# duanyiqun/DiffusionDepth

Hardware: NVIDIA H100
Metric: depth maps/sec @ KITTI 352x1216, Swin-L, 20 DDIM steps (higher is better)
Workload: dtype f32 (fp32-grade products on wgmma: 3-pass fp16 split, fp32 accumulate)

## Files before the change

### diffusiondepth_b200/csrc/convgen.cuh

```cuda
#pragma once
#include "conv_common.cuh"

namespace dd {

struct GenConvArgs {
  int B, H, W;
  int tiles_x, tiles_y, m_tiles, n_tiles;
  int kc0, kc1;
  int c0_ch;
  int taps;
  int ld_out, ch_off;
  int cout;
  const float* shift;
  float acc_scale;
  int relu;
  int m_valid;
  int stride;
  int add_first;
  int shuffle;
  float* y32;
  const float* add32;
  __half* out_hi;
  __half* out_lo;
  float split_scale;
  int* status;
};

constexpr int GEN_BK = 64;

template <int NT>
struct GenCfg {
  static constexpr int BK = GEN_BK;
  static constexpr int ROW_BYTES = BK * 2;
  static constexpr int A_BYTES = TILE_M * ROW_BYTES;
  static constexpr int B_BYTES = NT * ROW_BYTES;
  static constexpr int STAGE_BYTES = 2 * (A_BYTES + B_BYTES);
  static constexpr int NWG = NT > 128 ? 2 : 1;
  static constexpr int NW = NT / NWG;
  static constexpr int THREADS = 128 * (1 + NWG);
  static constexpr int LD = 20;
  static constexpr int STAGING_BYTES = NWG * 128 * LD * 4;
  static constexpr int STAGES_RAW = (227 * 1024 - 1024 - 512 - STAGING_BYTES) / STAGE_BYTES;
  static constexpr int STAGES = STAGES_RAW > 6 ? 6 : STAGES_RAW;
  static_assert(STAGES >= 2, "stage too large");
  static constexpr int SMEM_BYTES = STAGES * STAGE_BYTES + 1024 + 512 + STAGING_BYTES;
  static_assert(SMEM_BYTES <= 232448, "exceeds the 227 KB dynamic shared memory limit");
  static_assert(NW % 16 == 0 && NT <= 256, "bad N tile");
};

template <int NT>
__global__ void __launch_bounds__((GenCfg<NT>::THREADS), 1)
convgen_wgmma_kernel(const __grid_constant__ CUtensorMap tmA0_hi, const __grid_constant__ CUtensorMap tmA0_lo,
                     const __grid_constant__ CUtensorMap tmA1_hi, const __grid_constant__ CUtensorMap tmA1_lo,
                     const __grid_constant__ CUtensorMap tmB_hi, const __grid_constant__ CUtensorMap tmB_lo,
                     const GenConvArgs p) {
  using C = GenCfg<NT>;
  constexpr int NW = C::NW;
  extern __shared__ uint8_t smem_raw[];
  uint8_t* smem = reinterpret_cast<uint8_t*>((reinterpret_cast<uintptr_t>(smem_raw) + 1023) & ~uintptr_t(1023));
  uint64_t* full_bar = reinterpret_cast<uint64_t*>(smem + C::STAGES * C::STAGE_BYTES);
  uint64_t* empty_bar = full_bar + C::STAGES;
  float* stage_f = reinterpret_cast<float*>(smem + C::STAGES * C::STAGE_BYTES + 512);

  const int warp = threadIdx.x >> 5;
  const int lane = threadIdx.x & 31;
  const int kc_total = p.kc0 + p.kc1;
  const int k_iters = p.taps * kc_total;
  const int num_work = p.m_tiles * p.n_tiles;

  if (threadIdx.x == 0) {
    tma_prefetch_desc(&tmA0_hi);
    tma_prefetch_desc(&tmA0_lo);
    tma_prefetch_desc(&tmB_hi);
    tma_prefetch_desc(&tmB_lo);
    for (int s = 0; s < C::STAGES; ++s) {
      mbar_init(&full_bar[s], 2);
      mbar_init(&empty_bar[s], C::NWG);
    }
    fence_barrier_init();
  }
  __syncthreads();
  auto stage_ptr = [&](int s) { return smem + s * C::STAGE_BYTES; };

  if (warp < 4) {
    if constexpr (C::NWG > 1) setmaxnreg_dec<40>();
    if (warp == 0 || warp == 1) {
      const bool act = (warp == 0);
      const bool leader = elect_one();
      int stage = 0;
      uint32_t phase = 0;
      for (int work = blockIdx.x; work < num_work; work += gridDim.x) {
        const int nt = work % p.n_tiles;
        const int mt = work / p.n_tiles;
        const int tx = mt % p.tiles_x, ty = (mt / p.tiles_x) % p.tiles_y, img = mt / (p.tiles_x * p.tiles_y);
        const int x0 = tx * TILE_W, y0 = ty * TILE_H;
        for (int tap = 0; tap < p.taps; ++tap) {
          const int dy = p.taps == 9 ? tap / 3 - 1 : 0, dx = p.taps == 9 ? tap % 3 - 1 : 0;
          for (int kc = 0; kc < kc_total; ++kc) {
            mbar_wait(&empty_bar[stage], phase ^ 1);
            uint8_t* s = stage_ptr(stage);
            const int ax = x0 * p.stride + dx, ay = y0 * p.stride + dy;
            const int kw = kc < p.kc0 ? kc * C::BK : p.c0_ch + (kc - p.kc0) * C::BK;
            if (leader) {
              if (!act) {
                mbar_arrive_expect_tx(&full_bar[stage], 2 * C::B_BYTES);
                tma_load_3d(s + 2 * C::A_BYTES, &tmB_hi, &full_bar[stage], kw, nt * NT, tap);
                tma_load_3d(s + 2 * C::A_BYTES + C::B_BYTES, &tmB_lo, &full_bar[stage], kw, nt * NT, tap);
              } else if (kc < p.kc0) {
                mbar_arrive_expect_tx(&full_bar[stage], 2 * C::A_BYTES);
                tma_load_4d(s, &tmA0_hi, &full_bar[stage], kc * C::BK, ax, ay, img);
                tma_load_4d(s + C::A_BYTES, &tmA0_lo, &full_bar[stage], kc * C::BK, ax, ay, img);
              } else {
                mbar_arrive_expect_tx(&full_bar[stage], 2 * C::A_BYTES);
                tma_load_4d(s, &tmA1_hi, &full_bar[stage], (kc - p.kc0) * C::BK, ax, ay, img);
                tma_load_4d(s + C::A_BYTES, &tmA1_lo, &full_bar[stage], (kc - p.kc0) * C::BK, ax, ay, img);
              }
            }
            __syncwarp();
            if (++stage == C::STAGES) {
              stage = 0;
              phase ^= 1;
            }
          }
        }
      }
    }
  } else {
    if constexpr (C::NWG > 1) setmaxnreg_inc<232>();
    const int wg = (warp >> 2) - 1;
    const int t = threadIdx.x & 127;
    const int q = t >> 5;
    const int m = t;
    const int r = m >> 4, c = m & 15;
    float* S = stage_f + wg * 128 * C::LD;
    float* T = S + q * 32 * C::LD;
    const uint32_t b_off = static_cast<uint32_t>(wg * NW) * C::ROW_BYTES;
    int stage = 0;
    uint32_t phase = 0;
    bool overflow = false;
    const int cq = p.cout >> 2;
    float acc[2][NW / 2];
    for (int work = blockIdx.x; work < num_work; work += gridDim.x) {
      int prev = -1;
      for (int it = 0; it < k_iters; ++it) {
        mbar_wait(&full_bar[stage], phase);
        const uint32_t sa_hi = smem_u32(stage_ptr(stage));
        const uint32_t sa_lo = sa_hi + C::A_BYTES;
        const uint32_t sb_hi = sa_hi + 2 * C::A_BYTES + b_off;
        const uint32_t sb_lo = sb_hi + C::B_BYTES;
        wgmma_fence();
#pragma unroll
        for (int h = 0; h < 2; ++h) {
          const uint32_t ho = static_cast<uint32_t>(h * 64 * C::ROW_BYTES);
#pragma unroll
          for (int k = 0; k < C::BK / 16; ++k) {
            const uint64_t a_hi = wgmma_desc(sa_hi + ho + k * 32, C::ROW_BYTES);
            const uint64_t a_lo = wgmma_desc(sa_lo + ho + k * 32, C::ROW_BYTES);
            const uint64_t b_hi = wgmma_desc(sb_hi + k * 32, C::ROW_BYTES);
            const uint64_t b_lo = wgmma_desc(sb_lo + k * 32, C::ROW_BYTES);
            wgmma_f16<NW>(acc[h], a_lo, b_hi, (it | k) != 0 ? 1u : 0u);
            wgmma_f16<NW>(acc[h], a_hi, b_lo, 1u);
            wgmma_f16<NW>(acc[h], a_hi, b_hi, 1u);
          }
        }
        wgmma_commit();
        wgmma_wait<1>();
        mbar_arrive_if(&empty_bar[prev < 0 ? 0 : prev], t == 0 && prev >= 0);
        prev = stage;
        if (++stage == C::STAGES) {
          stage = 0;
          phase ^= 1;
        }
      }
      wgmma_wait<0>();
      wgmma_fence_regs(acc[0]);
      wgmma_fence_regs(acc[1]);
      mbar_arrive_if(&empty_bar[prev < 0 ? 0 : prev], t == 0 && prev >= 0);

      const int nt = work % p.n_tiles;
      const int mt = work / p.n_tiles;
      const int tx = mt % p.tiles_x, ty = (mt / p.tiles_x) % p.tiles_y, img = mt / (p.tiles_x * p.tiles_y);
      const int x = tx * TILE_W + c, y = ty * TILE_H + r;
      const bool valid = (x < p.W) && (y < p.H) && (p.m_valid <= 0 || (y * p.W + x) < p.m_valid);
      const uint32_t vmask = __ballot_sync(0xffffffffu, valid);
      const uint32_t row_base = static_cast<uint32_t>(((static_cast<size_t>(img) * p.H + y) * p.W + x) * p.cout);
      const uint32_t row_out = static_cast<uint32_t>(((static_cast<size_t>(img) * p.H + y) * p.W + x) * p.ld_out + p.ch_off);
      const bool xpose_path = (p.out_hi == nullptr);
#pragma unroll
      for (int ci = 0; ci < NW / 16; ++ci) {
        const int n0 = nt * NT + wg * NW + ci * 16;
        if (n0 >= p.cout) break;
        const int nvalid = p.cout - n0;
        named_bar_sync(2 + wg, 128);
        stage_acc_cols<NW, 16, C::LD>(acc[0], S, 0, ci * 2);
        stage_acc_cols<NW, 16, C::LD>(acc[1], S, 64, ci * 2);
        named_bar_sync(2 + wg, 128);
        uint32_t o_lane;
        if (p.shuffle) {
          const int sub = n0 / cq, cc = n0 - sub * cq;
          o_lane = static_cast<uint32_t>(
              ((static_cast<size_t>(img) * (2 * p.H) + (2 * y + (sub >> 1))) * (2 * p.W) + (2 * x + (sub & 1))) * cq + cc);
        } else {
          o_lane = row_base + static_cast<uint32_t>(n0);
        }
        const uint32_t o_out = p.shuffle ? o_lane : row_out + static_cast<uint32_t>(n0);
        if (xpose_path) {
          const int sl = lane & 3;
          const bool col_ok = 4 * sl < nvalid;
          const float4 sh = __ldg(reinterpret_cast<const float4*>(p.shift + n0) + sl);
          uint32_t o[4], oo[4];
          float4 ad[4];
#pragma unroll
          for (int k = 0; k < 4; ++k) {
            const int row = (lane >> 2) + 8 * k;
            o[k] = __shfl_sync(0xffffffffu, o_lane, row) + 4 * sl;
            oo[k] = __shfl_sync(0xffffffffu, o_out, row) + 4 * sl;
            ad[k] = (p.add32 && col_ok && ((vmask >> row) & 1u)) ? __ldg(reinterpret_cast<const float4*>(p.add32 + o[k]))
                                                                  : make_float4(0.f, 0.f, 0.f, 0.f);
          }
#pragma unroll
          for (int k = 0; k < 4; ++k) {
            const int row = (lane >> 2) + 8 * k;
            if (!((vmask >> row) & 1u) || !col_ok) continue;
            const float4 a4 = *reinterpret_cast<const float4*>(T + row * C::LD + 4 * sl);
            float tt[4] = {fmaf(a4.x, p.acc_scale, sh.x), fmaf(a4.y, p.acc_scale, sh.y), fmaf(a4.z, p.acc_scale, sh.z),
                           fmaf(a4.w, p.acc_scale, sh.w)};
            const float av[4] = {ad[k].x, ad[k].y, ad[k].z, ad[k].w};
#pragma unroll
            for (int j = 0; j < 4; ++j) {
              if (p.add_first) tt[j] += av[j];
              if (p.relu == 1) tt[j] = fmaxf(tt[j], 0.f);
              else if (p.relu == 2) tt[j] = 0.5f * tt[j] * (1.f + erff(tt[j] * 0.70710678118654752f));
              else if (p.relu == 3) tt[j] = tt[j] * fminf(fmaxf(tt[j] + 3.f, 0.f), 6.f) * (1.f / 6.f);
              if (!p.add_first) tt[j] += av[j];
            }
            if (p.y32) *reinterpret_cast<float4*>(p.y32 + oo[k]) = make_float4(tt[0], tt[1], tt[2], tt[3]);
          }
        } else if (valid) {
          float v[16];
#pragma unroll
          for (int j4 = 0; j4 < 4; ++j4) {
            const float4 sh = __ldg(reinterpret_cast<const float4*>(p.shift + n0) + j4);
            const float4 a4 = *reinterpret_cast<const float4*>(S + m * C::LD + 4 * j4);
// ... 9 lines not shown
                const float4 a = __ldg(reinterpret_cast<const float4*>(p.add32 + o_lane) + j4);
                v[4 * j4] += a.x; v[4 * j4 + 1] += a.y; v[4 * j4 + 2] += a.z; v[4 * j4 + 3] += a.w;
              }
            }
          }
          if (p.relu == 1) {
#pragma unroll
            for (int j = 0; j < 16; ++j) v[j] = fmaxf(v[j], 0.f);
          } else if (p.relu == 2) {
#pragma unroll
            for (int j = 0; j < 16; ++j) v[j] = 0.5f * v[j] * (1.f + erff(v[j] * 0.70710678118654752f));
          } else if (p.relu == 3) {
#pragma unroll
            for (int j = 0; j < 16; ++j) v[j] = v[j] * fminf(fmaxf(v[j] + 3.f, 0.f), 6.f) * (1.f / 6.f);
          }
          if (p.add32 && !p.add_first) {
#pragma unroll
            for (int j4 = 0; j4 < 4; ++j4) {
              if (4 * j4 < nvalid) {
                const float4 a = __ldg(reinterpret_cast<const float4*>(p.add32 + o_lane) + j4);
                v[4 * j4] += a.x; v[4 * j4 + 1] += a.y; v[4 * j4 + 2] += a.z; v[4 * j4 + 3] += a.w;
              }
            }
          }
          if (p.y32) {
            float4* d4 = reinterpret_cast<float4*>(p.y32 + o_out);
#pragma unroll
            for (int j = 0; j < 4; ++j)
              if (4 * j < nvalid) d4[j] = make_float4(v[4 * j], v[4 * j + 1], v[4 * j + 2], v[4 * j + 3]);
          }
          __align__(16) __half2 hi[8];
          __align__(16) __half2 lo[8];
          float amax = 0.f;
#pragma unroll
          for (int j = 0; j < 8; ++j) {
            const float s0 = v[2 * j] * p.split_scale, s1 = v[2 * j + 1] * p.split_scale;
            amax = fmaxf(amax, fmaxf(fabsf(s0), fabsf(s1)));
            hi[j] = __floats2half2_rn(s0, s1);
            const float2 back = __half22float2(hi[j]);
            lo[j] = __floats2half2_rn(s0 - back.x, s1 - back.y);
          }
          overflow |= !(amax <= 60000.f);
          uint4* dh = reinterpret_cast<uint4*>(p.out_hi + o_out);
          uint4* dl = reinterpret_cast<uint4*>(p.out_lo + o_out);
#pragma unroll
          for (int j = 0; j < 2; ++j) {
            if (8 * j < nvalid) {
              dh[j] = reinterpret_cast<const uint4*>(hi)[j];
              dl[j] = reinterpret_cast<const uint4*>(lo)[j];
            }
          }
        }
      }
    }
    if (overflow) atomicOr(p.status, 1);
  }
}

__global__ void nchw_to_nhwc_split_kernel(const float* __restrict__ in, __half* __restrict__ hi, __half* __restrict__ lo,
                                          int C, int P, float scale, int* status) {
  __shared__ float t[32][33];
  const int b = blockIdx.z;
  const int p0 = blockIdx.x * 32, c0 = blockIdx.y * 32;
  const float* src = in + static_cast<size_t>(b) * C * P;
  for (int i = threadIdx.y; i < 32; i += blockDim.y) {
    const int c = c0 + i, pp = p0 + threadIdx.x;
    t[i][threadIdx.x] = (c < C && pp < P) ? src[static_cast<size_t>(c) * P + pp] : 0.f;
  }
  __syncthreads();
  bool ov = false;
  for (int i = threadIdx.y; i < 32; i += blockDim.y) {
    const int pp = p0 + i, c = c0 + threadIdx.x;
    if (pp < P && c < C) {
      const float s = t[threadIdx.x][i] * scale;
      ov |= fabsf(s) > 60000.f;
      const __half h = __float2half_rn(s);
      const size_t o = (static_cast<size_t>(b) * P + pp) * C + c;
      hi[o] = h;
      lo[o] = __float2half_rn(s - __half2float(h));
    }
  }
  if (ov) atomicOr(status, 1);
}

__global__ void rgb_to_planes_kernel(const float* __restrict__ rgb, __half* __restrict__ hi, __half* __restrict__ lo,
                                     int B, int HW, float scale, int* status) {
  const size_t n = static_cast<size_t>(B) * HW;
  bool ov = false;
  for (size_t i = blockIdx.x * static_cast<size_t>(blockDim.x) + threadIdx.x; i < n * GEN_BK;
       i += static_cast<size_t>(gridDim.x) * blockDim.x) {
    const int c = static_cast<int>(i % GEN_BK);
    const size_t px = i / GEN_BK;
    float v = 0.f;
    if (c < 3) {
      const size_t b = px / HW, p = px % HW;
      v = rgb[(b * 3 + c) * HW + p] * scale;
    }
    ov |= fabsf(v) > 60000.f;
    const __half h = __float2half_rn(v);
    hi[i] = h;
    lo[i] = __float2half_rn(v - __half2float(h));
  }
  if (ov) atomicOr(status, 1);
}

__global__ void adaptive_avg_pool_nhwc_kernel(const float* __restrict__ in, float* __restrict__ out, int B, int IH, int IW,
// ... 65 lines not shown
```

### diffusiondepth_b200/csrc/engine.cu

```cuda
#include <cuda.h>
#include <cuda_runtime.h>
#include <math.h>
#include <stdio.h>
#include <stdlib.h>
#include <string.h>

#include <algorithm>
#include <map>
#include <string>
#include <vector>

#include "../../include/dd_engine.h"
#include "kernels.cuh"
#include "convgen.cuh"
#include "conv_halo.cuh"
#include "pred_fold.cuh"
#include "swin.cuh"
#include "mpvit.cuh"
#include "backward.cuh"

namespace {

thread_local std::string g_err;

// ... 1267 lines not shown
    if ((rc = bn_fold(bn, cout_conv, scale, shift, st))) return rc;
  } else if (bias) {
    CUDA_TRY(cudaMemcpyAsync(shift.data(), bias, cout_conv * 4, cudaMemcpyDeviceToHost, st));
    CUDA_TRY(cudaStreamSynchronize(st));
  }
  const int cp = cin_pad > 0 ? cin_pad : cin;
  L.cin = cp;
  L.taps = transposed ? 1 : taps;
  L.cout = transposed ? 4 * cout_conv : cout_conv;
  L.shuffle = transposed ? 1 : 0;
  L.relu = 1;
  L.nt = 64;
  if (nt > 0) {
    if (nt != 64 && nt != 128 && nt != 192 && nt != 256) return fail(DD_ERR_INVALID, "N tile must be 64, 128, 192 or 256");
    L.nt = nt;
  } else if (L.cout > 64) {
    int best = 1 << 30;
    for (int width : {256, 192, 128}) {
      const int padded = (L.cout + width - 1) / width * width;
      if (padded < best) { best = padded; L.nt = width; }
    }
  }
  if (L.cout % 8 != 0 || cp % 8 != 0) return fail(DD_ERR_UNSUPPORTED, "channels must be multiples of 8: " + name);
  const int cout_pad = (L.cout + L.nt - 1) / L.nt * L.nt;
  const size_t n = static_cast<size_t>(L.cout) * cp * L.taps;
  float* d_scale = nullptr;
  if ((rc = dev_alloc(owned, reinterpret_cast<void**>(&L.w_hi), n * 2))) return rc;
  if ((rc = dev_alloc(owned, reinterpret_cast<void**>(&L.w_lo), n * 2))) return rc;
  if ((rc = dev_alloc(owned, reinterpret_cast<void**>(&L.shift), cout_pad * 4))) return rc;
  if (bn) {
    if ((rc = dev_alloc(owned, reinterpret_cast<void**>(&d_scale), cout_conv * 4))) return rc;
    CUDA_TRY(cudaMemcpyAsync(d_scale, scale.data(), cout_conv * 4, cudaMemcpyHostToDevice, st));
  }
  if (cp != cin) {
    CUDA_TRY(cudaMemsetAsync(L.w_hi, 0, n * 2, st));
    CUDA_TRY(cudaMemsetAsync(L.w_lo, 0, n * 2, st));
  }
  std::vector<float> shift_full(cout_pad, 0.f);
  for (int i = 0; i < L.cout; ++i) shift_full[i] = shift[i % cout_conv];
  CUDA_TRY(cudaMemcpyAsync(L.shift, shift_full.data(), cout_pad * 4, cudaMemcpyHostToDevice, st));
  if (gen_parts(L.taps, gen_chunks(cp) + 1) > 1) {
    if ((rc = dev_alloc(owned, reinterpret_cast<void**>(&L.zero_shift), cout_pad * 4))) return rc;
    CUDA_TRY(cudaMemsetAsync(L.zero_shift, 0, cout_pad * 4, st));
  }
  const int nraw = static_cast<int>(static_cast<size_t>(cout_conv) * cin * (transposed ? 4 : taps));
  if ((rc = split_scale(scratch, st, &L.wscale, [&] {
         dd::absmax_scaled_kernel<<<absmax_grid(nraw), 256, 0, st>>>(w, d_scale, nraw, cin * L.taps, cout_conv,
                                                                     L.shuffle, scratch);
       })))
    return rc;
  dd::pack_gen_weight_kernel<<<256, 256, 0, st>>>(w, d_scale, L.w_hi, L.w_lo, L.cout, cin, L.taps, L.shuffle, L.wscale, cp);
  if ((rc = check_launch("pack_gen_weight"))) return rc;
  CUDA_TRY(cudaStreamSynchronize(st));
  if ((rc = make_weight_map(&L.mb_hi, L.w_hi, L.cout, cp, L.taps, dd::GEN_BK, L.nt))) return rc;
  if ((rc = make_weight_map(&L.mb_lo, L.w_lo, L.cout, cp, L.taps, dd::GEN_BK, L.nt))) return rc;
  L.alt = (L.nt == 256 && L.cout % 256 == 0 && L.cout % 192 == 0 && !L.shuffle);
  if (L.alt) {
    if ((rc = make_weight_map(&L.mb_hi_alt, L.w_hi, L.cout, cp, L.taps, dd::GEN_BK, 192))) return rc;
    if ((rc = make_weight_map(&L.mb_lo_alt, L.w_lo, L.cout, cp, L.taps, dd::GEN_BK, 192))) return rc;
  }
  return DD_OK;
}

int pack_gen(dd_engine* e, GenLayer& L, const std::string& wkey, const std::string& bnkey, int cin, int cout_conv,
             int taps, bool transposed, cudaStream_t st, float* scratch, int cin_pad = 0,
             const std::string& biaskey = std::string()) {
  const Raw* w = find(e, wkey);
  if (!w) return fail(DD_ERR_INVALID, "missing weights: " + wkey);
  const int k = taps == 9 ? 3 : (transposed ? 2 : 1);
  std::vector<int64_t> want = transposed ? std::vector<int64_t>{cin, cout_conv, 2, 2}
                                         : std::vector<int64_t>{cout_conv, cin, k, k};
  if (w->shape != want) return fail(DD_ERR_INVALID, "weight shape mismatch: " + wkey);
  const float* bn[4] = {nullptr, nullptr, nullptr, nullptr};
  const float* bias = nullptr;
  int rc;
  if (!bnkey.empty()) {
    if ((rc = find_bn(e, bnkey, bn))) return rc;
  } else if (!biaskey.empty()) {
    const Raw* b = find(e, biaskey);
    if (!b) return fail(DD_ERR_INVALID, "missing weights: " + biaskey);
    bias = b->ptr;
  }
  return pack_gen_weights(e, e->owned, L, w->ptr, wkey, bnkey.empty() ? nullptr : bn, bias, cin, cout_conv, taps,
                          transposed, cin_pad, 0, st, scratch);
}

int pack_linear(dd_engine* e, GenLayer& L, const std::string& wkey, const std::string& bkey, int N, int K,
                cudaStream_t st, float* scratch) {
  const Raw* w = find(e, wkey);
  if (!w) return fail(DD_ERR_INVALID, "missing weights: " + wkey);
  if (w->shape != std::vector<int64_t>{N, K}) return fail(DD_ERR_INVALID, "weight shape mismatch: " + wkey);
  const Raw* b = nullptr;
  if (!bkey.empty() && !(b = find(e, bkey))) return fail(DD_ERR_INVALID, "missing weights: " + bkey);
  return pack_gen_weights(e, e->owned, L, w->ptr, wkey, nullptr, b ? b->ptr : nullptr, K, N, 1, false, 0, 0, st,
                          scratch);
}

int pack_producers(dd_engine* e, cudaStream_t st, float* scratch) {
  Producers& p = e->prod;
  int rc;
  for (int i = 0; i < p.nlev; ++i) {
    const std::string si = std::to_string(i);
    if (p.neck) {
      const std::string h = "hahineck.";
      if ((rc = pack_gen(e, p.lat[i], h + "lateral_convs." + si + ".conv.weight", h + "lateral_convs." + si + ".bn",
                         p.C[i], p.C[i], 1, false, st, scratch))) return rc;
      const std::string pj = i == 0 ? h + "conv_proj.0" : h + "trans_proj." + std::to_string(i - 1);
      const std::string fs = i == 0 ? h + "conv_fusion.0" : h + "trans_fusion." + std::to_string(i - 1);
      if ((rc = pack_gen(e, p.proj[i], pj + ".conv.weight", pj + ".bn", p.C[i], 512, 1, false, st, scratch))) return rc;
      if ((rc = pack_gen(e, p.fus[i], fs + ".conv.weight", fs + ".bn", p.C[i] + 512, p.C[i], 9, false, st, scratch))) return rc;
    }
    if ((rc = pack_gen(e, p.fl[i], "conv_lateral." + si + ".0.weight", "conv_lateral." + si + ".1", p.C[i], 256, 9, false,
// ... 74 lines not shown
    return launched(e, "convgen");
  };
  int rc;
  if (parts == 1) {
    if ((rc = make_act_map(&m[0], a0.hi, g.B, sh, sw, c0, dd::GEN_BK, L.stride))) return rc;
    if ((rc = make_act_map(&m[1], a0.lo, g.B, sh, sw, c0, dd::GEN_BK, L.stride))) return rc;
    if (c1 > 0) {
      if ((rc = make_act_map(&m[2], a1.hi, g.B, g.H, g.W, c1, dd::GEN_BK))) return rc;
      if ((rc = make_act_map(&m[3], a1.lo, g.B, g.H, g.W, c1, dd::GEN_BK))) return rc;
    } else {
      m[2] = m[0];
      m[3] = m[1];
    }
    m[4] = use_alt ? L.mb_hi_alt : L.mb_hi;
    m[5] = use_alt ? L.mb_lo_alt : L.mb_lo;
    return launch(a);
  }
  if (add32 || L.shuffle || !partial || !L.zero_shift)
    return fail(DD_ERR_UNSUPPORTED, "producer conv deeper than one accumulator takes, with an addend or no partial buffer");
  const int kc_total = a.kc0 + a.kc1, per = (kc_total + parts - 1) / parts;
  for (int p = 0; p * per < kc_total; ++p) {
    const int ka = p * per, kb = std::min(kc_total, ka + per);
    const int s0a = std::min(ka, a.kc0), s0b = std::min(kb, a.kc0);
    const int s1a = std::max(ka, a.kc0) - a.kc0, s1b = std::max(kb, a.kc0) - a.kc0;
    const int w0 = std::min(s0b * dd::GEN_BK, c0) - s0a * dd::GEN_BK;
    const int w1 = std::min(s1b * dd::GEN_BK, c1) - s1a * dd::GEN_BK;
    dd::GenConvArgs ap = a;
    int wcol, wlen;
    if (w0 > 0) {
      if ((rc = make_act_map(&m[0], a0.hi + s0a * dd::GEN_BK, g.B, sh, sw, w0, dd::GEN_BK, L.stride, c0))) return rc;
      if ((rc = make_act_map(&m[1], a0.lo + s0a * dd::GEN_BK, g.B, sh, sw, w0, dd::GEN_BK, L.stride, c0))) return rc;
      ap.kc0 = s0b - s0a;
      ap.c0_ch = w0;
      wcol = s0a * dd::GEN_BK;
      wlen = w0 + w1;
    } else {
      ap.kc0 = 0;
      ap.c0_ch = (c0 + s1a * dd::GEN_BK) % dd::GEN_BK;
      wcol = c0 + s1a * dd::GEN_BK - ap.c0_ch;
      wlen = ap.c0_ch + w1;
    }
    ap.kc1 = s1b - s1a;
    if (w1 > 0) {
      if ((rc = make_act_map(&m[2], a1.hi + s1a * dd::GEN_BK, g.B, g.H, g.W, w1, dd::GEN_BK, 1, c1))) return rc;
      if ((rc = make_act_map(&m[3], a1.lo + s1a * dd::GEN_BK, g.B, g.H, g.W, w1, dd::GEN_BK, 1, c1))) return rc;
    }
    if (w0 == 0) {
      m[0] = m[2];
      m[1] = m[3];
    } else if (w1 == 0) {
      m[2] = m[0];
      m[3] = m[1];
    }
    if ((rc = make_weight_map(&m[4], L.w_hi + wcol, L.cout, wlen, L.taps, dd::GEN_BK, nt, L.cin))) return rc;
    if ((rc = make_weight_map(&m[5], L.w_lo + wcol, L.cout, wlen, L.taps, dd::GEN_BK, nt, L.cin))) return rc;
    const bool last = kb == kc_total;
    ap.relu = last ? act : 0;
    ap.shift = last ? L.shift : L.zero_shift;
    ap.add_first = 1;
    ap.add32 = p > 0 ? partial : nullptr;
    ap.y32 = last ? y32 : partial;
    ap.out_hi = last ? a.out_hi : nullptr;
    ap.out_lo = last ? a.out_lo : nullptr;
    ap.ld_out = last ? a.ld_out : L.cout;
    ap.ch_off = last ? ch_off : 0;
    if ((rc = launch(ap))) return rc;
  }
  return DD_OK;
}

int run_gen(dd_engine* e, const GenLayer& L, const Planes& a0, int c0, const Planes& a1, int c1, int H, int W,
            float* y32, const float* add32, const Planes* out, cudaStream_t st, int src_h = 0, int src_w = 0,
            int ld_out = 0, int ch_off = 0) {
  return launch_gen(e, L, L.relu, {e->cfg.batch, H, W, 0, src_h, src_w}, a0, c0, a1, c1, y32, add32, out, ld_out, ch_off,
                    st, 0, nullptr, e->prod.KS);
}

int pack_resnet(dd_engine* e, cudaStream_t st, float* scratch) {
  ResNetW& r = e->rn;
  int rc;
  for (int s = 0; s < 4; ++s) {
    r.blocks[s].assign(r.depths[s], ResBlockW());
    const int cprev = s == 0 ? 3 : r.C[s - 1];
    for (int b = 0; b < r.depths[s]; ++b) {
      ResBlockW& W = r.blocks[s][b];
      const std::string bp = "backbone.layers." + std::to_string(s) + "." + std::to_string(b) + ".";
      const int cin = b == 0 ? cprev : r.C[s];
      const int pad = (cin % dd::GEN_BK) ? dd::GEN_BK : 0;
      if ((rc = pack_gen(e, W.c1, bp + "conv1.weight", bp + "bn1", cin, r.C[s], 9, false, st, scratch, pad))) return rc;
      W.c1.stride = b == 0 ? 2 : 1;
      if ((rc = pack_gen(e, W.c2, bp + "conv2.weight", bp + "bn2", r.C[s], r.C[s], 9, false, st, scratch))) return rc;
      W.c2.add_first = 1;
      W.has_ds = (b == 0);
      if (W.has_ds) {
        if ((rc = pack_gen(e, W.ds, bp + "downsample.weight", "", cin, r.C[s], 9, false, st, scratch, pad,
                           bp + "downsample.bias"))) return rc;
        W.ds.stride = 2;
        W.ds.relu = 0;
      }
    }
  }
  r.ready = true;
  return DD_OK;
}

int run_resnet(dd_engine* e, const float* rgb, float* const* feats_out, cudaStream_t st) {
  ResNetW& r = e->rn;
  const int B = e->cfg.batch;
// ... 1229 lines not shown
  if (!h->weights_ready || !(swin || resnet || mpvit)) return fail(DD_ERR_INVALID, "backbone not enabled / weights not finalized");
  auto run = [&](const float* img, float* const* outs, cudaStream_t s) {
    return swin ? run_swin(h, img, outs, s) : (resnet ? run_resnet(h, img, outs, s) : run_mpvit(h, img, outs, s));
  };
  cudaStream_t st = static_cast<cudaStream_t>(cuda_stream);
  CUDA_TRY(cudaSetDevice(h->cfg.device));
  int rc;
  if ((rc = bind_workspace(h, workspace, workspace_bytes))) return rc;
  CUDA_TRY(cudaMemsetAsync(h->status, 0, 64, st));
  h->launches = 0;
  bool want_out = false;
  for (int i = 0; feats_out && i < 4; ++i) want_out |= (feats_out[i] != nullptr);
  if ((h->cfg.flags & DD_FLAG_CUDA_GRAPH) && !want_out) {
    const size_t n = static_cast<size_t>(h->cfg.batch) * 3 *
                     (swin ? h->bb.H * h->bb.W : (resnet ? h->rn.H * h->rn.W : h->mp.H * h->mp.W));
    CUDA_TRY(cudaMemcpyAsync(h->rgb_stage, rgb, n * 4, cudaMemcpyDeviceToDevice, st));
    if ((rc = graph_run(h, dd_engine::G_BACKBONE, st, [&](cudaStream_t s) { return run(h->rgb_stage, nullptr, s); }))) return rc;
  } else if ((rc = run(rgb, feats_out, st))) {
    return rc;
  }
  h->feats_ready = true;
  return DD_OK;
}

int dd_bench_gemm(dd_handle h, int32_t M, int32_t K, int32_t N, int32_t mode, int32_t iters, float* ms_out) {
  if (!h || !ms_out || M < 1 || K % dd::GEN_BK || N % 192 && N % 256) return fail(DD_ERR_INVALID, "bad argument");
  CUDA_TRY(cudaSetDevice(h->cfg.device));
  cudaStream_t st = h->cap_stream;
  const size_t Mp = (static_cast<size_t>(M) + 127) / 128 * 128 + 128;
  Planes A, O;
  GenLayer L;
  float *y = nullptr, *bias = nullptr;
  int* status = nullptr;
  CUDA_TRY(cudaMalloc(&A.hi, Mp * K * 2));
  CUDA_TRY(cudaMalloc(&A.lo, Mp * K * 2));
  CUDA_TRY(cudaMalloc(&O.hi, Mp * N * 2));
  CUDA_TRY(cudaMalloc(&O.lo, Mp * N * 2));
  CUDA_TRY(cudaMalloc(&y, Mp * N * 4));
  CUDA_TRY(cudaMalloc(&L.w_hi, static_cast<size_t>(N) * K * 2));
  CUDA_TRY(cudaMalloc(&L.w_lo, static_cast<size_t>(N) * K * 2));
  CUDA_TRY(cudaMalloc(&bias, N * 4));
  CUDA_TRY(cudaMalloc(&status, 64));
  CUDA_TRY(cudaMemsetAsync(A.hi, 0x11, Mp * K * 2, st));
  CUDA_TRY(cudaMemsetAsync(A.lo, 0x01, Mp * K * 2, st));
  CUDA_TRY(cudaMemsetAsync(L.w_hi, 0x11, static_cast<size_t>(N) * K * 2, st));
  CUDA_TRY(cudaMemsetAsync(L.w_lo, 0x01, static_cast<size_t>(N) * K * 2, st));
  CUDA_TRY(cudaMemsetAsync(bias, 0, N * 4, st));
  CUDA_TRY(cudaMemsetAsync(y, 0, Mp * N * 4, st));
  L.cin = K;
  L.cout = N;
  L.nt = (N % 256 == 0) ? 256 : 192;
  L.shift = bias;
  int rc;
  if ((rc = make_weight_map(&L.mb_hi, L.w_hi, N, K, 1, dd::GEN_BK, L.nt))) return rc;
  if ((rc = make_weight_map(&L.mb_lo, L.w_lo, N, K, 1, dd::GEN_BK, L.nt))) return rc;
  int* saved = h->status;
  h->status = status;
  if ((rc = time_per_call(st, 3, iters, ms_out, [&]() {
         return run_gemm(h, L, A, M, mode == 2 ? 2 : 0, (mode == 0 || mode == 1) ? y : nullptr, mode == 1 ? y : nullptr,
                         mode == 2 ? &O : nullptr, st);
       })))
    return rc;
  h->status = saved;
  for (void* p : {(void*)A.hi, (void*)A.lo, (void*)O.hi, (void*)O.lo, (void*)y, (void*)L.w_hi, (void*)L.w_lo, (void*)bias, (void*)status})
    cudaFree(p);
  return DD_OK;
}

int dd_encode(dd_handle h, const float* depth, int32_t height, int32_t width, float* latent_out, void* cuda_stream) {
  if (!h || !depth || !latent_out) return fail(DD_ERR_INVALID, "null argument");
  if (!h->weights_ready || !h->enc_w1) return fail(DD_ERR_INVALID, "encoder weights (depth_transform.conv_transform.*) not registered");
  if ((height + 1) / 2 != h->cfg.latent_h || (width + 1) / 2 != h->cfg.latent_w)
    return fail(DD_ERR_INVALID, "depth map size does not match the engine's latent grid");
  cudaStream_t st = static_cast<cudaStream_t>(cuda_stream);
  CUDA_TRY(cudaSetDevice(h->cfg.device));
  dd::EncoderArgs a;
  a.depth = depth;
  a.w1 = h->enc_w1;
  a.b1 = h->enc_b1;
  a.w2 = h->enc_w2;
  a.b2 = h->enc_b2;
  a.out = latent_out;
  a.H = height;
  a.W = width;
  a.h = h->cfg.latent_h;
  a.w = h->cfg.latent_w;
  dim3 grid((a.w + 15) / 16, (a.h + 15) / 16, h->cfg.batch);
  dd::encoder_kernel<<<grid, 256, 0, st>>>(a);
  return check_launch("encoder");
}

int64_t dd_last_launch_count(dd_handle h) { return h ? h->launches : 0; }

int dd_poll_status(dd_handle h, void* cuda_stream) {
  if (!h) return fail(DD_ERR_INVALID, "null handle");
  if (!h->status) return DD_OK;
  CUDA_TRY(cudaSetDevice(h->cfg.device));
  return poll_status(h, static_cast<cudaStream_t>(cuda_stream));
}

size_t dd_conv3x3_workspace_bytes(int32_t batch, int32_t cin, int32_t cout, int32_t height, int32_t width) {
  const size_t BP = static_cast<size_t>(batch) * height * width;
  const size_t nw = static_cast<size_t>(cin) * cout * 9;
  size_t off = 0;
  auto add = [&](size_t bytes) { off = align_up(off, 1024) + bytes; };
  add(64);
  add(BP * cin * 4);
  add(BP * cin * 2);
// ... 350 lines not shown
```

### diffusiondepth_b200/csrc/ptx.cuh

```cuda
#pragma once
#include <cuda.h>
#include <cuda_fp16.h>
#include <stdint.h>

namespace dd {

__device__ __forceinline__ uint32_t smem_u32(const void* p) {
  return static_cast<uint32_t>(__cvta_generic_to_shared(p));
}

__device__ __forceinline__ bool elect_one() {
  uint32_t pred = 0;
  asm volatile(
      "{\n\t.reg .pred P;\n\t"
      "elect.sync _|P, 0xffffffff;\n\t"
      "selp.u32 %0, 1, 0, P;\n\t}\n"
      : "=r"(pred));
  return pred != 0;
}

__device__ __forceinline__ void mbar_init(uint64_t* bar, uint32_t count) {
  asm volatile("mbarrier.init.shared::cta.b64 [%0], %1;" ::"r"(smem_u32(bar)), "r"(count));
}
__device__ __forceinline__ void fence_barrier_init() {
// ... 160 lines not shown
      : "l"(a), "l"(b), "r"(acc));
}

__device__ __forceinline__ uint64_t wgmma_desc_mn(uint32_t smem_addr, uint32_t mn_stride) {
  uint64_t d = 0;
  d |= static_cast<uint64_t>((smem_addr & 0x3FFFFu) >> 4);
  d |= static_cast<uint64_t>((mn_stride & 0x3FFFFu) >> 4) << 16;
  d |= static_cast<uint64_t>(1024u >> 4) << 32;
  d |= static_cast<uint64_t>(1) << 62;
  return d;
}

template <int N>
__device__ __forceinline__ void wgmma_f16_mn(float (&d)[N / 2], uint64_t a, uint64_t b);

template <>
__device__ __forceinline__ void wgmma_f16_mn<64>(float (&d)[32], uint64_t a, uint64_t b) {
  asm volatile(
      "{\n\t.reg .pred p;\n\tsetp.ne.b32 p, 1, 0;\n\t"
      "wgmma.mma_async.sync.aligned.m64n64k16.f32.f16.f16 {%0, %1, %2, %3, %4, %5, %6, %7, %8, %9, %10, %11, %12, %13, %14, %15, %16, %17, %18, %19, %20, %21, %22, %23, %24, %25, %26, %27, %28, %29, %30, %31}, %32, %33, p, 1, 1, 1, 1;\n\t}\n"
      : "+f"(d[0]), "+f"(d[1]), "+f"(d[2]), "+f"(d[3]), "+f"(d[4]), "+f"(d[5]), "+f"(d[6]), "+f"(d[7]), "+f"(d[8]), "+f"(d[9]), "+f"(d[10]), "+f"(d[11]), "+f"(d[12]), "+f"(d[13]), "+f"(d[14]), "+f"(d[15]), "+f"(d[16]), "+f"(d[17]), "+f"(d[18]), "+f"(d[19]), "+f"(d[20]), "+f"(d[21]), "+f"(d[22]), "+f"(d[23]), "+f"(d[24]), "+f"(d[25]), "+f"(d[26]), "+f"(d[27]), "+f"(d[28]), "+f"(d[29]), "+f"(d[30]), "+f"(d[31])
      : "l"(a), "l"(b));
}

template <>
__device__ __forceinline__ void wgmma_f16_mn<128>(float (&d)[64], uint64_t a, uint64_t b) {
  asm volatile(
      "{\n\t.reg .pred p;\n\tsetp.ne.b32 p, 1, 0;\n\t"
      "wgmma.mma_async.sync.aligned.m64n128k16.f32.f16.f16 {%0, %1, %2, %3, %4, %5, %6, %7, %8, %9, %10, %11, %12, %13, %14, %15, %16, %17, %18, %19, %20, %21, %22, %23, %24, %25, %26, %27, %28, %29, %30, %31, %32, %33, %34, %35, %36, %37, %38, %39, %40, %41, %42, %43, %44, %45, %46, %47, %48, %49, %50, %51, %52, %53, %54, %55, %56, %57, %58, %59, %60, %61, %62, %63}, %64, %65, p, 1, 1, 1, 1;\n\t}\n"
      : "+f"(d[0]), "+f"(d[1]), "+f"(d[2]), "+f"(d[3]), "+f"(d[4]), "+f"(d[5]), "+f"(d[6]), "+f"(d[7]), "+f"(d[8]), "+f"(d[9]), "+f"(d[10]), "+f"(d[11]), "+f"(d[12]), "+f"(d[13]), "+f"(d[14]), "+f"(d[15]), "+f"(d[16]), "+f"(d[17]), "+f"(d[18]), "+f"(d[19]), "+f"(d[20]), "+f"(d[21]), "+f"(d[22]), "+f"(d[23]), "+f"(d[24]), "+f"(d[25]), "+f"(d[26]), "+f"(d[27]), "+f"(d[28]), "+f"(d[29]), "+f"(d[30]), "+f"(d[31]), "+f"(d[32]), "+f"(d[33]), "+f"(d[34]), "+f"(d[35]), "+f"(d[36]), "+f"(d[37]), "+f"(d[38]), "+f"(d[39]), "+f"(d[40]), "+f"(d[41]), "+f"(d[42]), "+f"(d[43]), "+f"(d[44]), "+f"(d[45]), "+f"(d[46]), "+f"(d[47]), "+f"(d[48]), "+f"(d[49]), "+f"(d[50]), "+f"(d[51]), "+f"(d[52]), "+f"(d[53]), "+f"(d[54]), "+f"(d[55]), "+f"(d[56]), "+f"(d[57]), "+f"(d[58]), "+f"(d[59]), "+f"(d[60]), "+f"(d[61]), "+f"(d[62]), "+f"(d[63])
      : "l"(a), "l"(b));
}

template <int N>
__device__ __forceinline__ void wgmma_e4m3(float (&d)[N / 2], uint64_t a, uint64_t b, uint32_t acc);

template <>
__device__ __forceinline__ void wgmma_e4m3<128>(float (&d)[64], uint64_t a, uint64_t b, uint32_t acc) {
  asm volatile(
      "{\n\t.reg .pred p;\n\tsetp.ne.b32 p, %66, 0;\n\t"
      "wgmma.mma_async.sync.aligned.m64n128k32.f32.e4m3.e4m3 {%0, %1, %2, %3, %4, %5, %6, %7, %8, %9, %10, %11, %12, %13, %14, %15, %16, %17, %18, %19, %20, %21, %22, %23, %24, %25, %26, %27, %28, %29, %30, %31, %32, %33, %34, %35, %36, %37, %38, %39, %40, %41, %42, %43, %44, %45, %46, %47, %48, %49, %50, %51, %52, %53, %54, %55, %56, %57, %58, %59, %60, %61, %62, %63}, %64, %65, p, 1, 1;\n\t}\n"
      : "+f"(d[0]), "+f"(d[1]), "+f"(d[2]), "+f"(d[3]), "+f"(d[4]), "+f"(d[5]), "+f"(d[6]), "+f"(d[7]), "+f"(d[8]), "+f"(d[9]), "+f"(d[10]), "+f"(d[11]), "+f"(d[12]), "+f"(d[13]), "+f"(d[14]), "+f"(d[15]), "+f"(d[16]), "+f"(d[17]), "+f"(d[18]), "+f"(d[19]), "+f"(d[20]), "+f"(d[21]), "+f"(d[22]), "+f"(d[23]), "+f"(d[24]), "+f"(d[25]), "+f"(d[26]), "+f"(d[27]), "+f"(d[28]), "+f"(d[29]), "+f"(d[30]), "+f"(d[31]), "+f"(d[32]), "+f"(d[33]), "+f"(d[34]), "+f"(d[35]), "+f"(d[36]), "+f"(d[37]), "+f"(d[38]), "+f"(d[39]), "+f"(d[40]), "+f"(d[41]), "+f"(d[42]), "+f"(d[43]), "+f"(d[44]), "+f"(d[45]), "+f"(d[46]), "+f"(d[47]), "+f"(d[48]), "+f"(d[49]), "+f"(d[50]), "+f"(d[51]), "+f"(d[52]), "+f"(d[53]), "+f"(d[54]), "+f"(d[55]), "+f"(d[56]), "+f"(d[57]), "+f"(d[58]), "+f"(d[59]), "+f"(d[60]), "+f"(d[61]), "+f"(d[62]), "+f"(d[63])
      : "l"(a), "l"(b), "r"(acc));
}

template <int R>
__device__ __forceinline__ void setmaxnreg_dec() { asm volatile("setmaxnreg.dec.sync.aligned.u32 %0;" ::"n"(R)); }
template <int R>
__device__ __forceinline__ void setmaxnreg_inc() { asm volatile("setmaxnreg.inc.sync.aligned.u32 %0;" ::"n"(R)); }

__device__ __forceinline__ void named_bar_sync(int id, int count) {
  asm volatile("bar.sync %0, %1;" ::"r"(id), "r"(count) : "memory");
}

template <int N, int CH, int LD>
__device__ __forceinline__ void stage_acc_cols(const float (&d)[N / 2], float* S, int row0, int c0_blk) {
  const int t = threadIdx.x & 127;
  const int r = row0 + 16 * (t >> 5) + ((t & 31) >> 2);
  const int c = 2 * (t & 3);
#pragma unroll
  for (int i = 0; i < CH / 8; ++i) {
    const int blk = c0_blk + i;
    S[r * LD + 8 * i + c] = d[4 * blk];
    S[r * LD + 8 * i + c + 1] = d[4 * blk + 1];
    S[(r + 8) * LD + 8 * i + c] = d[4 * blk + 2];
    S[(r + 8) * LD + 8 * i + c + 1] = d[4 * blk + 3];
  }
}

}
```

Baseline: 25.89.

## Ping-pong two consumer warpgroups over N-units so epilogue overlaps the next MMA

```diff
diff --git a/diffusiondepth_b200/csrc/convgen.cuh b/diffusiondepth_b200/csrc/convgen.cuh
--- a/diffusiondepth_b200/csrc/convgen.cuh
+++ b/diffusiondepth_b200/csrc/convgen.cuh
@@ -28,21 +28,23 @@
 
 constexpr int GEN_BK = 64;
 
+constexpr int gen_unit_cols(int nt) { return nt > 128 ? nt / 2 : nt; }
+
 template <int NT>
 struct GenCfg {
   static constexpr int BK = GEN_BK;
   static constexpr int ROW_BYTES = BK * 2;
+  static constexpr int NW = gen_unit_cols(NT);
+  static constexpr int UNITS = NT / NW;
   static constexpr int A_BYTES = TILE_M * ROW_BYTES;
-  static constexpr int B_BYTES = NT * ROW_BYTES;
+  static constexpr int B_BYTES = NW * ROW_BYTES;
   static constexpr int STAGE_BYTES = 2 * (A_BYTES + B_BYTES);
-  static constexpr int NWG = NT > 128 ? 2 : 1;
-  static constexpr int NW = NT / NWG;
-  static constexpr int THREADS = 128 * (1 + NWG);
+  static constexpr int THREADS = 384;
   static constexpr int LD = 20;
-  static constexpr int STAGING_BYTES = NWG * 128 * LD * 4;
+  static constexpr int STAGING_BYTES = 2 * 128 * LD * 4;
   static constexpr int STAGES_RAW = (227 * 1024 - 1024 - 512 - STAGING_BYTES) / STAGE_BYTES;
   static constexpr int STAGES = STAGES_RAW > 6 ? 6 : STAGES_RAW;
-  static_assert(STAGES >= 2, "stage too large");
+  static_assert(STAGES >= 3, "stage too large");
   static constexpr int SMEM_BYTES = STAGES * STAGE_BYTES + 1024 + 512 + STAGING_BYTES;
   static_assert(SMEM_BYTES <= 232448, "exceeds the 227 KB dynamic shared memory limit");
   static_assert(NW % 16 == 0 && NT <= 256, "bad N tile");
@@ -75,7 +77,7 @@
     tma_prefetch_desc(&tmB_lo);
     for (int s = 0; s < C::STAGES; ++s) {
       mbar_init(&full_bar[s], 2);
-      mbar_init(&empty_bar[s], C::NWG);
+      mbar_init(&empty_bar[s], 1);
     }
     fence_barrier_init();
   }
@@ -83,7 +85,7 @@
   auto stage_ptr = [&](int s) { return smem + s * C::STAGE_BYTES; };
 
   if (warp < 4) {
-    if constexpr (C::NWG > 1) setmaxnreg_dec<40>();
+    setmaxnreg_dec<40>();
     if (warp == 0 || warp == 1) {
       const bool act = (warp == 0);
       const bool leader = elect_one();
@@ -94,6 +96,7 @@
         const int mt = work / p.n_tiles;
         const int tx = mt % p.tiles_x, ty = (mt / p.tiles_x) % p.tiles_y, img = mt / (p.tiles_x * p.tiles_y);
         const int x0 = tx * TILE_W, y0 = ty * TILE_H;
+        for (int u = 0; u < C::UNITS; ++u) {
         for (int tap = 0; tap < p.taps; ++tap) {
           const int dy = p.taps == 9 ? tap / 3 - 1 : 0, dx = p.taps == 9 ? tap % 3 - 1 : 0;
           for (int kc = 0; kc < kc_total; ++kc) {
@@ -104,8 +107,8 @@
             if (leader) {
               if (!act) {
                 mbar_arrive_expect_tx(&full_bar[stage], 2 * C::B_BYTES);
-                tma_load_3d(s + 2 * C::A_BYTES, &tmB_hi, &full_bar[stage], kw, nt * NT, tap);
-                tma_load_3d(s + 2 * C::A_BYTES + C::B_BYTES, &tmB_lo, &full_bar[stage], kw, nt * NT, tap);
+                tma_load_3d(s + 2 * C::A_BYTES, &tmB_hi, &full_bar[stage], kw, nt * NT + u * C::NW, tap);
+                tma_load_3d(s + 2 * C::A_BYTES + C::B_BYTES, &tmB_lo, &full_bar[stage], kw, nt * NT + u * C::NW, tap);
               } else if (kc < p.kc0) {
                 mbar_arrive_expect_tx(&full_bar[stage], 2 * C::A_BYTES);
                 tma_load_4d(s, &tmA0_hi, &full_bar[stage], kc * C::BK, ax, ay, img);
@@ -123,10 +126,11 @@
             }
           }
         }
+        }
       }
     }
   } else {
-    if constexpr (C::NWG > 1) setmaxnreg_inc<232>();
+    setmaxnreg_inc<232>();
     const int wg = (warp >> 2) - 1;
     const int t = threadIdx.x & 127;
     const int q = t >> 5;
@@ -134,19 +138,22 @@
     const int r = m >> 4, c = m & 15;
     float* S = stage_f + wg * 128 * C::LD;
     float* T = S + q * 32 * C::LD;
-    const uint32_t b_off = static_cast<uint32_t>(wg * NW) * C::ROW_BYTES;
-    int stage = 0;
-    uint32_t phase = 0;
     bool overflow = false;
     const int cq = p.cout >> 2;
     float acc[2][NW / 2];
+    int unit = -1;
     for (int work = blockIdx.x; work < num_work; work += gridDim.x) {
+    for (int u = 0; u < C::UNITS; ++u) {
+      if (((++unit) & 1) != wg) continue;
+      if (unit > 0) named_bar_sync(4 + wg, 256);
+      int stage = (unit * k_iters) % C::STAGES;
+      uint32_t phase = ((unit * k_iters) / C::STAGES) & 1;
       int prev = -1;
       for (int it = 0; it < k_iters; ++it) {
         mbar_wait(&full_bar[stage], phase);
         const uint32_t sa_hi = smem_u32(stage_ptr(stage));
         const uint32_t sa_lo = sa_hi + C::A_BYTES;
-        const uint32_t sb_hi = sa_hi + 2 * C::A_BYTES + b_off;
+        const uint32_t sb_hi = sa_hi + 2 * C::A_BYTES;
         const uint32_t sb_lo = sb_hi + C::B_BYTES;
         wgmma_fence();
 #pragma unroll
@@ -172,6 +179,8 @@
           phase ^= 1;
         }
       }
+      if (u + 1 < C::UNITS || work + static_cast<int>(gridDim.x) < num_work)
+        named_bar_arrive(4 + (wg ^ 1), 256);
       wgmma_wait<0>();
       wgmma_fence_regs(acc[0]);
       wgmma_fence_regs(acc[1]);
@@ -188,7 +197,7 @@
       const bool xpose_path = (p.out_hi == nullptr);
 #pragma unroll
       for (int ci = 0; ci < NW / 16; ++ci) {
-        const int n0 = nt * NT + wg * NW + ci * 16;
+        const int n0 = nt * NT + u * NW + ci * 16;
         if (n0 >= p.cout) break;
         const int nvalid = p.cout - n0;
         named_bar_sync(2 + wg, 128);
@@ -304,6 +313,7 @@
           }
         }
       }
+    }
     }
     if (overflow) atomicOr(p.status, 1);
   }
diff --git a/diffusiondepth_b200/csrc/engine.cu b/diffusiondepth_b200/csrc/engine.cu
--- a/diffusiondepth_b200/csrc/engine.cu
+++ b/diffusiondepth_b200/csrc/engine.cu
@@ -1343,12 +1343,12 @@
   dd::pack_gen_weight_kernel<<<256, 256, 0, st>>>(w, d_scale, L.w_hi, L.w_lo, L.cout, cin, L.taps, L.shuffle, L.wscale, cp);
   if ((rc = check_launch("pack_gen_weight"))) return rc;
   CUDA_TRY(cudaStreamSynchronize(st));
-  if ((rc = make_weight_map(&L.mb_hi, L.w_hi, L.cout, cp, L.taps, dd::GEN_BK, L.nt))) return rc;
-  if ((rc = make_weight_map(&L.mb_lo, L.w_lo, L.cout, cp, L.taps, dd::GEN_BK, L.nt))) return rc;
+  if ((rc = make_weight_map(&L.mb_hi, L.w_hi, L.cout, cp, L.taps, dd::GEN_BK, dd::gen_unit_cols(L.nt)))) return rc;
+  if ((rc = make_weight_map(&L.mb_lo, L.w_lo, L.cout, cp, L.taps, dd::GEN_BK, dd::gen_unit_cols(L.nt)))) return rc;
   L.alt = (L.nt == 256 && L.cout % 256 == 0 && L.cout % 192 == 0 && !L.shuffle);
   if (L.alt) {
-    if ((rc = make_weight_map(&L.mb_hi_alt, L.w_hi, L.cout, cp, L.taps, dd::GEN_BK, 192))) return rc;
-    if ((rc = make_weight_map(&L.mb_lo_alt, L.w_lo, L.cout, cp, L.taps, dd::GEN_BK, 192))) return rc;
+    if ((rc = make_weight_map(&L.mb_hi_alt, L.w_hi, L.cout, cp, L.taps, dd::GEN_BK, dd::gen_unit_cols(192)))) return rc;
+    if ((rc = make_weight_map(&L.mb_lo_alt, L.w_lo, L.cout, cp, L.taps, dd::GEN_BK, dd::gen_unit_cols(192)))) return rc;
   }
   return DD_OK;
 }
@@ -1529,8 +1529,8 @@
       m[2] = m[0];
       m[3] = m[1];
     }
-    if ((rc = make_weight_map(&m[4], L.w_hi + wcol, L.cout, wlen, L.taps, dd::GEN_BK, nt, L.cin))) return rc;
-    if ((rc = make_weight_map(&m[5], L.w_lo + wcol, L.cout, wlen, L.taps, dd::GEN_BK, nt, L.cin))) return rc;
+    if ((rc = make_weight_map(&m[4], L.w_hi + wcol, L.cout, wlen, L.taps, dd::GEN_BK, dd::gen_unit_cols(nt), L.cin))) return rc;
+    if ((rc = make_weight_map(&m[5], L.w_lo + wcol, L.cout, wlen, L.taps, dd::GEN_BK, dd::gen_unit_cols(nt), L.cin))) return rc;
     const bool last = kb == kc_total;
     ap.relu = last ? act : 0;
     ap.shift = last ? L.shift : L.zero_shift;
@@ -2866,8 +2866,8 @@
   L.nt = (N % 256 == 0) ? 256 : 192;
   L.shift = bias;
   int rc;
-  if ((rc = make_weight_map(&L.mb_hi, L.w_hi, N, K, 1, dd::GEN_BK, L.nt))) return rc;
-  if ((rc = make_weight_map(&L.mb_lo, L.w_lo, N, K, 1, dd::GEN_BK, L.nt))) return rc;
+  if ((rc = make_weight_map(&L.mb_hi, L.w_hi, N, K, 1, dd::GEN_BK, dd::gen_unit_cols(L.nt)))) return rc;
+  if ((rc = make_weight_map(&L.mb_lo, L.w_lo, N, K, 1, dd::GEN_BK, dd::gen_unit_cols(L.nt)))) return rc;
   int* saved = h->status;
   h->status = status;
   if ((rc = time_per_call(st, 3, iters, ms_out, [&]() {
diff --git a/diffusiondepth_b200/csrc/ptx.cuh b/diffusiondepth_b200/csrc/ptx.cuh
--- a/diffusiondepth_b200/csrc/ptx.cuh
+++ b/diffusiondepth_b200/csrc/ptx.cuh
@@ -236,6 +236,9 @@
 __device__ __forceinline__ void named_bar_sync(int id, int count) {
   asm volatile("bar.sync %0, %1;" ::"r"(id), "r"(count) : "memory");
 }
+__device__ __forceinline__ void named_bar_arrive(int id, int count) {
+  asm volatile("bar.arrive %0, %1;" ::"r"(id), "r"(count) : "memory");
+}
 
 template <int N, int CH, int LD>
 __device__ __forceinline__ void stage_acc_cols(const float (&d)[N / 2], float* S, int row0, int c0_blk) {
diff --git a/profiles/producer_ab.py b/profiles/producer_ab.py
--- /dev/null
+++ b/profiles/producer_ab.py
@@ -0,0 +1,244 @@
+#!/usr/bin/env python
+import argparse
+import json
+import os
+import re
+import subprocess
+import sys
+import tempfile
+
+ROOT = os.path.dirname(os.path.dirname(os.path.abspath(__file__)))
+B, IH, IW = 4, 352, 1216
+E, DEPTHS = 192, (2, 2, 18, 2)
+GEN_BK, SPLIT_ITERS = 64, 110
+
+
+def cdiv(a, b):
+    return (a + b - 1) // b
+
+
+def c3_launches():
+    out = []
+    hs, ws = [cdiv(IH, 4)], [cdiv(IW, 4)]
+    for _ in range(3):
+        hs.append(cdiv(hs[-1], 2))
+        ws.append(cdiv(ws[-1], 2))
+
+    def gemm(layer, fam, M, N, K):
+        out.append(dict(layer=layer, family=fam, M=M, N=N, K=K, taps=1, conv=None, kc=cdiv(K, GEN_BK)))
+
+    def conv(layer, fam, s, N, cin, taps):
+        kc = cdiv(cin, GEN_BK)
+        parts = cdiv(taps * kc, SPLIT_ITERS)
+        per = cdiv(kc, parts)
+        for p in range(parts):
+            ka, kb = p * per, min(kc, p * per + per)
+            if ka >= kc:
+                break
+            name = layer + (f" part {p + 1}/{parts}" if parts > 1 else "")
+            out.append(dict(layer=name, family=fam, M=B * hs[s] * ws[s], N=N, K=taps * cin, taps=taps,
+                            conv=(hs[s], ws[s]), kc=kb - ka))
+
+    for s in range(4):
+        C, M = E << s, B * hs[s] * ws[s]
+        for k in range(DEPTHS[s]):
+            gemm(f"s{s}.b{k}.qkv", f"swin s{s} qkv", M, 3 * C, C)
+            gemm(f"s{s}.b{k}.proj", f"swin s{s} proj", M, C, C)
+            gemm(f"s{s}.b{k}.fc1", f"swin s{s} fc1", M, 4 * C, C)
+            gemm(f"s{s}.b{k}.fc2", f"swin s{s} fc2", M, C, 4 * C)
+        if s < 3:
+            gemm(f"s{s}.reduction", f"swin s{s} merge", B * hs[s + 1] * ws[s + 1], 2 * C, 4 * C)
+    for i in range(4):
+        C = E << i
+        conv(f"neck.lat{i}", "neck lateral", i, C, C, 1)
+        conv(f"neck.proj{i}", "neck proj", i, 512, C, 1)
+        conv(f"neck.fus{i}", "neck fusion", i, C, C + 512, 9)
+    for i in range(3, -1, -1):
+        conv(f"fpn.lat{i}", "fpn lateral", i, 256, E << i, 9)
+        if i > 0:
+            conv(f"fpn.up{i - 1}", "fpn up", i, 1024, 256, 1)
+    return out
+
+
+def m_tiles(L):
+    if L["conv"] is None:
+        return cdiv(L["M"], 128)
+    h, w = L["conv"]
+    return B * cdiv(h, 8) * cdiv(w, 16)
+
+
+def profile_rows(out_dir=None):
+    sys.path.insert(0, ROOT)
+    sys.path.insert(0, os.path.join(ROOT, "tests"))
+    import torch
+    from torch.profiler import ProfilerActivity, profile as tprofile
+    import dd_helpers
+    from oracle import configs, restate
+
+    dev = torch.device("cuda:0")
+    model = dd_helpers.build_mirror("swinl", 20).to(dev)
+    model.depth_head.use_cuda_graph = False
+    sample = {k: v.to(dev) for k, v in restate.synthetic_sample(B, IH, IW, configs.SEED_INPUTS).items()}
+    with torch.no_grad():
+        for _ in range(2):
+            model(sample)
+        torch.cuda.synchronize()
+        with tprofile(activities=[ProfilerActivity.CUDA]) as prof:
+            model(sample)
+            torch.cuda.synchronize()
+    with tempfile.TemporaryDirectory() as td:
+        path = os.path.join(td, "trace.json")
+        prof.export_chrome_trace(path)
+        with open(path) as f:
+            trace = json.load(f)
+    kern = sorted((e for e in trace["traceEvents"] if e.get("cat") == "kernel"), key=lambda e: e["ts"])
+    total_ms = sum(e["dur"] for e in kern) / 1e3
+    gen = [e for e in kern if "convgen_wgmma_kernel" in e["name"]]
+    layers = c3_launches()
+    if len(gen) != len(layers):
+        raise SystemExit(f"{len(gen)} convgen launches, expected {len(layers)}: the launch order changed")
+    rows = []
+    for L, ev in zip(layers, gen):
+        nt = int(re.search(r"convgen_wgmma_kernel<(\d+)>", ev["name"]).group(1))
+        work = m_tiles(L) * cdiv(L["N"], nt)
+        ms = ev["dur"] / 1e3
+        kc, kc_total = L["kc"], cdiv(L["K"] // L["taps"], GEN_BK)
+        flops = 2.0 * L["M"] * L["N"] * L["K"] * kc / kc_total
+        parts = cdiv(L["taps"] * kc_total, SPLIT_ITERS)
+        rows.append(dict(layer=L["layer"], family=L["family"], M=L["M"], N=L["N"], K=L["K"], taps=L["taps"],
+                         k_iters=L["taps"] * kc, nt=nt, work=work, grid=ev["args"]["grid"][0], parts=parts, ms=ms,
+                         tflops=flops / (ms * 1e-3) / 1e12, flops=flops))
+    res = {"gpu": torch.cuda.get_device_name(0), "forward_kernel_ms": total_ms, "rows": rows}
+    if out_dir:
+        os.makedirs(out_dir, exist_ok=True)
+        with open(os.path.join(out_dir, "producer_profile.json"), "w") as f:
+            json.dump(res, f, indent=1)
+    return res
+
+
+def families(rows):
+    fam = {}
+    for r in rows:
+        f = fam.setdefault(r["family"], {"launches": 0, "ms": 0.0, "flops": 0.0})
+        f["launches"] += 1
+        f["ms"] += r["ms"]
+        f["flops"] += r["flops"]
+    return fam
+
+
+def print_profile(res):
+    rows = res["rows"]
+    gen_ms = sum(r["ms"] for r in rows)
+    gen_fl = sum(r["flops"] for r in rows)
+    print(f"{res['gpu']}: one C3 forward, profiler on, no CUDA graph: {res['forward_kernel_ms']:.1f} ms of kernel time; "
+          f"convgen_wgmma_kernel {gen_ms:.2f} ms in {len(rows)} launches, {gen_fl / 1e12:.3f} TFLOP, "
+          f"{gen_fl / (gen_ms * 1e-3) / 1e12:.1f} TFLOP/s")
+    print(f"{'layer':<24} {'M x N x K':>22} {'taps':>4} {'kit':>4} {'NT':>4} {'work':>6} {'grid':>5} {'parts':>5} "
+          f"{'ms':>8} {'TF/s':>7}")
+    for r in rows:
+        print(f"{r['layer']:<24} {r['M']:>8} x {r['N']:>4} x {r['K']:>5} {r['taps']:>4} {r['k_iters']:>4} {r['nt']:>4} "
+              f"{r['work']:>6} {r['grid']:>5} {r['parts']:>5} {r['ms']:8.3f} {r['tflops']:7.1f}")
+    print(f"\n{'family':<18} {'launches':>8} {'ms':>8} {'TF/s':>7}")
+    for name, f in families(rows).items():
+        print(f"{name:<18} {f['launches']:>8} {f['ms']:8.3f} {f['flops'] / (f['ms'] * 1e-3) / 1e12:7.1f}")
+
+
+def worker(iters, warmup):
+    sys.path.insert(0, ROOT)
+    sys.path.insert(0, os.path.join(ROOT, "tests"))
+    import torch
+    import dd_helpers
+    from diffusiondepth_b200 import lib_path
+    from diffusiondepth_b200.engine import DenoiseEngine
+    from oracle import configs, restate
+
+    if not torch.cuda.is_available():
+        raise SystemExit("producer_ab.py times kernels on an H100; there is no CPU path")
+    dev = torch.device("cuda:0")
+    model = dd_helpers.build_mirror("swinl", 20).to(dev)
+    sample = {k: v.to(dev) for k, v in restate.synthetic_sample(B, IH, IW, configs.SEED_INPUTS).items()}
+    seen = {}
+    orig = DenoiseEngine.run_backbone
+
+    def spy(self, rgb, want_feats=False):
+        seen["eng"], seen["rgb"] = self, rgb
+        return orig(self, rgb, want_feats)
+
+    DenoiseEngine.run_backbone = spy
+    with torch.no_grad():
+        model(sample)
+    DenoiseEngine.run_backbone = orig
+    eng, rgb = seen["eng"], seen["rgb"]
+
+    def chain():
+        eng.run_backbone(rgb)
+        eng.build_condition(None)
+
+    for _ in range(warmup):
+        chain()
+    torch.cuda.synchronize()
+    t0, t1 = torch.cuda.Event(enable_timing=True), torch.cuda.Event(enable_timing=True)
+    t0.record()
+    for _ in range(iters):
+        chain()
+    t1.record()
+    t1.synchronize()
+    eng.poll_status()
+    print(json.dumps({"lib": lib_path(), "gpu": torch.cuda.get_device_name(0), "ms": t0.elapsed_time(t1) / iters}),
+          flush=True)
+
+
+def ab(libs, rounds, iters, warmup):
+    def run(path, *args):
+        env = dict(os.environ, DD_ENGINE_LIB=os.path.abspath(path))
+        out = subprocess.run([sys.executable, os.path.abspath(__file__), *args], env=env, cwd=ROOT, check=True,
+                             stdout=subprocess.PIPE, text=True).stdout
+        return json.loads(out.strip().splitlines()[-1])
+
+    runs = {name: [] for name, _ in libs}
+    for _ in range(rounds):
+        for name, path in libs:
+            runs[name].append(run(path, "--worker", "--iters", str(iters), "--warmup", str(warmup))["ms"])
+    prof = {name: run(path, "--profile-json") for name, path in libs}
+    base = libs[0][0]
+    print(f"producer chain (dd_run_backbone + dd_build_condition, graphed), ms per call, {rounds} alternating rounds "
+          f"of {iters}:")
+    for name, _ in libs:
+        ms = sorted(runs[name])
+        med, bmed = ms[len(ms) // 2], sorted(runs[base])[len(ms) // 2]
+        print(f"  {name:>8}: {' '.join(f'{m:.2f}' for m in runs[name])}  median {med:.2f} "
+              f"({100 * (med / bmed - 1):+.1f} % vs {base})")
+    print("\nconvgen_wgmma_kernel per layer family (profiled forward, ms):")
+    fams = {name: families(prof[name]["rows"]) for name, _ in libs}
+    print(f"{'family':<18} " + " ".join(f"{n:>10}" for n, _ in libs))
+    for fam in fams[base]:
+        print(f"{fam:<18} " + " ".join(f"{fams[n][fam]['ms']:10.3f}" for n, _ in libs))
+    print(f"{'total':<18} " + " ".join(f"{sum(f['ms'] for f in fams[n].values()):10.3f}" for n, _ in libs))
+    print(json.dumps({"gpu": prof[base]["gpu"], "chain_ms": runs,
+                      "families": {n: {k: v["ms"] for k, v in fams[n].items()} for n, _ in libs}}))
+
+
+def main():
+    ap = argparse.ArgumentParser()
+    ap.add_argument("--lib", action="append", default=[], metavar="NAME=PATH", help="library to time (repeatable)")
+    ap.add_argument("--rounds", type=int, default=3)
+    ap.add_argument("--iters", type=int, default=20)
+    ap.add_argument("--warmup", type=int, default=3)
+    ap.add_argument("--profile", action="store_true")
+    ap.add_argument("--out", default=None, help="profile mode: directory for producer_profile.json")
+    ap.add_argument("--worker", action="store_true", help=argparse.SUPPRESS)
+    ap.add_argument("--profile-json", action="store_true", help=argparse.SUPPRESS)
+    args = ap.parse_args()
+    if args.worker:
+        return worker(args.iters, args.warmup)
+    if args.profile_json:
+        return print(json.dumps(profile_rows()))
+    if args.profile:
+        return print_profile(profile_rows(args.out))
+    libs = [tuple(s.split("=", 1)) for s in args.lib] or [("current", os.path.join(ROOT, "diffusiondepth_b200",
+                                                                                    "libddengine.so"))]
+    ab(libs, args.rounds, args.iters, args.warmup)
+
+
+if __name__ == "__main__":
+    main()
```

Result: faster. 27.04, median of 6 (+4.4%).
